# aynik/carta1

Hardware: AMD Instinct MI355X
Metric: atrac1_stereo_frames_per_s_encode (higher is better)
Workload: dtype f32+f64

## Files before the change

### carta1_amd/capi.py

```python
import ctypes as C
import os

HERE = os.path.dirname(os.path.abspath(__file__))
LIB_PATH = os.environ.get('C1_LIB') or os.path.join(HERE, 'lib', 'libcarta1_hip.so')

FRAME = 512
UNIT_BYTES = 212
SIGNAL_WHITE = 0
SIGNAL_PINK_BURSTS = 1
SIGNAL_MIXED = 2
SIGNAL_PARTIALS = 3


class Carta1Error(RuntimeError):
    def __init__(self, code, message):
        super().__init__('carta1_hip error %d: %s' % (code, message))
        self.code = code


class Tables(C.Structure):
    _fields_ = [('scale_factors', C.c_double * 64), ('window_short', C.c_double * 32),
                ('mdct_fwd64', C.c_double * 32), ('mdct_fwd256', C.c_double * 128),
                ('mdct_fwd512', C.c_double * 256), ('mdct_inv64', C.c_double * 32),
                ('mdct_inv256', C.c_double * 128), ('mdct_inv512', C.c_double * 256),
# ... 38 lines not shown
    'c1_dec_stream_create': (C.c_int, [C.c_void_p, C.c_int, C.POINTER(C.c_void_p)]),
    'c1_dec_stream_push': (C.c_int, [C.c_void_p, C.c_void_p, C.c_int64, C.POINTER(C.c_void_p)]),
    'c1_dec_stream_destroy': (C.c_int, [C.c_void_p]),
    'c1_generate_device': (C.c_int, [C.c_void_p, C.c_int, C.c_uint32, C.c_int64, C.c_void_p]),
    'c1_pcm_from_int_device': (C.c_int, [C.c_void_p, C.c_void_p, C.c_int, C.c_int, C.c_int64, C.POINTER(C.c_void_p)]),
    'c1_pcm_to_int16_device': (C.c_int, [C.c_void_p, C.POINTER(C.c_void_p), C.c_int, C.c_int64, C.c_void_p]),
    'c1_host_alloc': (C.c_int, [C.c_size_t, C.POINTER(C.c_void_p)]),
    'c1_host_free': (C.c_int, [C.c_void_p]),
    'c1_table_fast_paths': (C.c_int, [C.POINTER(C.c_int), C.POINTER(C.c_int)]),
    'c1_encode_wav_batch': (C.c_int, [C.c_void_p, C.c_void_p, C.c_int, C.c_int, C.c_int64, C.POINTER(EncodeOptions), C.c_void_p]),
    'c1_decode_wav16_batch': (C.c_int, [C.c_void_p, C.c_void_p, C.c_int, C.c_int64, C.c_void_p]),
    'c1_aea_header': (C.c_int, [C.c_char_p, C.c_uint32, C.c_int, C.c_void_p]),
    'c1_encode_stages_device': (C.c_int, [C.c_void_p, C.POINTER(C.c_void_p), C.c_int, C.c_int64, C.c_int,
                                          C.POINTER(EncodeOptions), C.c_void_p, C.c_void_p, C.c_void_p,
                                          C.c_void_p]),
    'c1_detect_stages_device': (C.c_int, [C.c_void_p, C.POINTER(C.c_void_p), C.c_int, C.c_int64, C.c_int,
                                          C.POINTER(EncodeOptions), C.c_void_p, C.c_void_p]),
    'c1_libm_device': (C.c_int, [C.c_void_p, C.c_int, C.c_void_p, C.c_void_p, C.c_int64]),
    'c1_detect_scores_device': (C.c_int, [C.c_void_p, C.POINTER(C.c_void_p), C.c_int, C.c_int64, C.c_int,
                                          C.POINTER(EncodeOptions), C.c_int, C.c_void_p, C.c_void_p, C.c_void_p]),
    'c1_detect_spec_mags_device': (C.c_int, [C.c_void_p, C.POINTER(C.c_void_p), C.c_int, C.c_int64, C.c_int, C.c_void_p, C.c_void_p]),
    'c1_log2f_error_device': (C.c_int, [C.c_void_p, C.c_uint32, C.c_uint64, C.POINTER(C.c_double)]),
    'c1_ctx_detection_stats': (C.c_int, [C.c_void_p, C.POINTER(C.c_uint64), C.POINTER(C.c_uint64)]),
    'c1_alloc_bounds_device': (C.c_int, [C.c_void_p, C.c_void_p, C.c_int64, C.c_void_p, C.c_void_p]),
    'c1_spec_stages_device': (C.c_int, [C.c_void_p, C.POINTER(C.c_void_p), C.c_int, C.c_int64, C.c_int,
                                        C.POINTER(EncodeOptions), C.c_void_p, C.c_void_p, C.c_void_p]),
    'c1_quantize': (C.c_int, [C.c_void_p, C.c_void_p, C.c_int, C.c_int, C.c_int, C.c_void_p]),
    'c1_dequantize': (C.c_int, [C.c_void_p, C.c_void_p, C.c_int, C.c_int, C.c_int, C.c_void_p]),
    'c1_fft': (C.c_int, [C.c_void_p, C.c_void_p, C.c_void_p, C.c_int, C.c_void_p]),
    'c1_qmf_analysis_batch': (C.c_int, [C.c_void_p, C.c_void_p, C.c_int64, C.c_int, C.c_void_p]),
    'c1_mdct_batch': (C.c_int, [C.c_void_p, C.c_void_p, C.c_int64, C.c_int, C.c_void_p, C.c_void_p, C.c_void_p]),
    'c1_unpack_units': (C.c_int, [C.c_void_p, C.c_void_p, C.c_int64, C.c_void_p, C.c_void_p, C.c_void_p, C.c_void_p, C.c_void_p]),
    'c1_dequantize_frames': (C.c_int, [C.c_void_p, C.c_int64, C.c_void_p, C.c_void_p, C.c_void_p, C.c_void_p, C.c_void_p, C.c_void_p]),
    'c1_imdct_batch': (C.c_int, [C.c_void_p, C.c_void_p, C.c_int64, C.c_int, C.c_void_p, C.c_void_p]),
    'c1_qmf_synthesis_batch': (C.c_int, [C.c_void_p, C.c_void_p, C.c_int64, C.c_int, C.c_void_p]),
    'c1_select_block_modes': (C.c_int, [C.c_void_p, C.c_void_p, C.c_int64, C.c_int, C.c_double, C.c_void_p]),
    'c1_quantize_frames': (C.c_int, [C.c_void_p, C.c_void_p, C.c_int64, C.c_void_p, C.c_void_p, C.c_void_p, C.c_void_p,
                                     C.c_void_p, C.c_void_p]),
    'c1_pack_spec_tap_device': (C.c_int, [C.c_void_p, C.c_void_p, C.c_void_p, C.c_void_p, C.c_void_p, C.c_int64, C.c_int,
                                          C.c_void_p, C.c_void_p]),
}

_lib = None


def load():
# ... 38 lines not shown
```

### carta1_amd/codec.py

```python
import ctypes as C
import math
import struct

import numpy as np

from . import capi

AEA_HEADER_SIZE = 2048
AEA_MAGIC = bytes([0x00, 0x08, 0x00, 0x00])
AEA_TITLE_OFFSET, AEA_TITLE_SIZE = 4, 256
AEA_FRAME_COUNT_OFFSET, AEA_CHANNEL_COUNT_OFFSET = 260, 264
BFU_AMOUNTS = (20, 28, 32, 36, 40, 44, 48, 52)
SPECS_PER_BFU = (8, 8, 8, 8, 4, 4, 4, 4, 8, 8, 8, 8, 6, 6, 6, 6, 6, 6, 6, 6, 6, 6, 6, 6, 7, 7, 7, 7, 9, 9, 9, 9,
                 10, 10, 10, 10, 12, 12, 12, 12, 12, 12, 12, 12, 20, 20, 20, 20, 20, 20, 20, 20)
WORD_LENGTH_BITS = (0, 2, 3, 4, 5, 6, 7, 8, 9, 10, 11, 12, 13, 14, 15, 16)


_BIASED = None


def packaged_biased_table(bias):
    global _BIASED
    if _BIASED is None:
        import json
# ... 81 lines not shown
        capi.check(capi.load().c1_ctx_kernel_ms(self._h, name.encode(), C.byref(ms), C.byref(n)))
        return ms.value, n.value

    def set_speculation(self, mode):
        capi.check(capi.load().c1_ctx_set_speculation(self._h, int(mode)))

    def set_decode_precision(self, binary32):
        capi.check(capi.load().c1_ctx_set_decode_precision(self._h, 1 if binary32 else 0))

    def speculation_stats(self, reset=False):
        u, r = C.c_uint64(0), C.c_uint64(0)
        capi.check(capi.load().c1_ctx_speculation_stats(self._h, C.byref(u), C.byref(r), 1 if reset else 0))
        return u.value, r.value

    def speculation_deferred(self):
        u = C.c_uint64(0)
        capi.check(capi.load().c1_ctx_speculation_deferred(self._h, C.byref(u)))
        return int(u.value)

    def quantization_stats(self):
        u, r = C.c_uint64(0), C.c_uint64(0)
        capi.check(capi.load().c1_ctx_quantization_stats(self._h, C.byref(u), C.byref(r)))
        return int(u.value), int(r.value)

    def detection_stats(self):
        u, r = C.c_uint64(0), C.c_uint64(0)
        capi.check(capi.load().c1_ctx_detection_stats(self._h, C.byref(u), C.byref(r)))
        return int(u.value), int(r.value)

    def encode(self, channels, options=None, halo_frames=0, out=None):
        opts = (options or EncoderOptions()).to_c()
        chans = [np.ascontiguousarray(c, dtype=np.float32) for c in channels]
        n = len(chans[0])
        if any(len(c) != n for c in chans) or n % 512:
            raise ValueError('channels must have equal length, a multiple of 512')
        frames = n // 512 - halo_frames
        if out is None:
            units = np.zeros((max(frames, 0) * len(chans), 212), dtype=np.uint8)
        else:
            units = out
            if units.dtype != np.uint8 or not units.flags['C_CONTIGUOUS'] or units.size != max(frames, 0) * len(chans) * 212:
                raise ValueError('out must be a contiguous uint8 array of frames * channels * 212 bytes')
            units = units.reshape(-1, 212)
        ptrs = capi.ptr_array([c.ctypes.data + halo_frames * 512 * 4 for c in chans])
        capi.check(capi.load().c1_encode_batch(self._h, ptrs, len(chans), frames, halo_frames, C.byref(opts),
                                               units.ctypes.data))
# ... 430 lines not shown
```

### carta1_amd/csrc/c1_api.hip

```cpp
#include <algorithm>
#include <cmath>
#include <cstdarg>
#include <cstdio>
#include <cstdlib>
#include <cstring>
#include <map>
#include <memory>
#include <atomic>
#include <mutex>
#include <string>
#include <thread>
#include <vector>

#include "c1_internal.h"
#include "c1_detect_bound.h"

#pragma clang fp contract(off)

namespace {

#include "c1_default_tables.inc"

thread_local std::string g_error;
int fail(int code, const char *fmt, ...) {
// ... 270 lines not shown
      for (int wl = 0; wl < 15; wl++) order.push_back(s * 16 + wl);
    std::sort(order.begin(), order.end(), [&](int x, int y) { return d->rank[x] < d->rank[y]; });
    for (int A = 1; A <= 12 && !d->rank_affine; A++)
      for (int B = 1; B <= 36 && !d->rank_affine; B++)
        for (int C = -2 * B; C <= 0 && !d->rank_affine; C++) {
          auto key = [&](int idx) { const int s = idx >> 4, wl = idx & 15; return wl == 0 ? A * s + C : A * s - B * wl - B; };
          bool ok = true;
          int lo = key(order[0]), hi = lo;
          for (size_t i = 1; i < order.size() && ok; i++) {
            const int k0 = key(order[i - 1]), k1 = key(order[i]);
            const bool req = d->rank[order[i]] == d->rank[order[i - 1]];
            if (req ? (k1 != k0) : !(k1 > k0)) ok = false;
            lo = std::min(lo, k1); hi = std::max(hi, k1);
          }
          if (ok && hi - lo + 1 < 1023) {
            d->rank_affine = 1; d->rank_a = A; d->rank_b = B; d->rank_c = C; d->rank_off = 1 - lo;
          }
        }
  }
  return C1_OK;
}

constexpr int kTotals = 8;
constexpr int64_t kSpecMinUnits = 64;
constexpr int kListHead = 8;
constexpr int64_t kMaxChunkFrames = (int64_t)1 << 27;

struct Timing {
  hipEvent_t start, stop;
  int kind;
};
enum { K_ANALYSIS = 0, K_ALLOCATE, K_PACK, K_DECODE, K_REDO, K_KINDS };
const char *const kKindNames[K_KINDS] = {"analysis", "allocate", "pack", "decode", "redo"};

}

struct c1_ctx {
  std::recursive_mutex mu;
  int device = 0;
  hipStream_t stream = nullptr;
  bool own_stream = false;
  C1DevTables *d_tables = nullptr;
  C1DevEncOpts *d_opts = nullptr;
  c1_encode_options last_opts;
  bool have_opts = false;
  int64_t ws_units = 0;
  float *d_coefs[2] = {nullptr, nullptr};
  uint8_t *d_side[2] = {nullptr, nullptr};
  uint8_t *d_alloc[2] = {nullptr, nullptr};
  uint8_t *d_cand[2] = {nullptr, nullptr};
  uint32_t *d_work[2] = {nullptr, nullptr};
  float *d_eps[2] = {nullptr, nullptr};
  uint32_t *d_redo[2] = {nullptr, nullptr};
  unsigned long long *d_spec_totals = nullptr;
  int spec_mode = 1;
  float spec_defer = 1.0f;
  bool decode_binary32 = false;
  bool spec_tables_ok = false;
  int64_t det_units = 0;
  float *d_bands[2] = {nullptr, nullptr};
  double *d_feat[2] = {nullptr, nullptr};
  uint8_t *d_modes[2] = {nullptr, nullptr};
  uint32_t *d_lists[2] = {nullptr, nullptr};
  bool overlap = false;
  hipStream_t s_tail = nullptr;
  hipEvent_t ev_main[2] = {nullptr, nullptr}, ev_tail[2] = {nullptr, nullptr};
  bool tail_used[2] = {false, false};
  bool tail_pending = false;
  int ws_next = 0;
  int64_t chunk_frames = 0;
  bool pipeline = true;
  hipStream_t s_ana = nullptr, s_rest = nullptr;
  hipEvent_t ev_in = nullptr, ev_ana[2] = {nullptr, nullptr}, ev_free[2] = {nullptr, nullptr}, ev_end[2] = {nullptr, nullptr};
  int timing_depth = 0;
  bool profiling = false;
  std::vector<Timing> timings;
  std::vector<hipEvent_t> event_pool;
  double ms[K_KINDS] = {0, 0, 0, 0, 0};
  int launches[K_KINDS] = {0, 0, 0, 0, 0};
// ... 113 lines not shown
}
void bind_defer(c1_ctx *ctx, int p, C1EncodeLaunch *L) {
  L->defer_list = ctx->d_redo[p] + kListHead + 3 * (size_t)ctx->ws_units;
}

int ensure_io(c1_ctx *ctx, size_t bytes) {
  if (bytes <= ctx->d_io_bytes) return C1_OK;
  if (ctx->d_io) hipFree(ctx->d_io);
  ctx->d_io = nullptr; ctx->d_io_bytes = 0;
  HIP_TRY(hipMalloc(&ctx->d_io, bytes));
  ctx->d_io_bytes = bytes;
  return C1_OK;
}

int upload_opts(c1_ctx *ctx, const c1_encode_options *opts) {
  if (!opts) return fail(C1_ERR_ARG, "options are NULL");
  if (ctx->have_opts && memcmp(&ctx->last_opts, opts, sizeof *opts) == 0) return C1_OK;
  C1DevEncOpts h;
  const int rc = build_encode_opts(*opts, &h);
  if (rc) return rc;
  int jr = join_tail(ctx);
  if (jr) return jr;
  HIP_TRY(hipStreamSynchronize(ctx->stream));
  HIP_TRY(hipMemcpy(ctx->d_opts, &h, sizeof h, hipMemcpyHostToDevice));
  ctx->last_opts = *opts;
  ctx->have_opts = true;
  return C1_OK;
}

hipEvent_t take_event(c1_ctx *ctx) {
  if (!ctx->event_pool.empty()) {
    hipEvent_t e = ctx->event_pool.back();
    ctx->event_pool.pop_back();
    return e;
  }
  hipEvent_t e;
  hipEventCreateWithFlags(&e, hipEventDisableSystemFence);
  return e;
}
struct ScopedTiming {
  c1_ctx *ctx;
  Timing t;
  bool on;
  hipStream_t stream;
  ScopedTiming(c1_ctx *c, int kind, hipStream_t s = nullptr) : ctx(c), on(c->profiling), stream(s ? s : c->stream) {
    if (!on) return;
// ... 77 lines not shown
    HIP_TRY(hipStreamWaitEvent(sA, ctx->ev_in, 0));
    HIP_TRY(hipStreamWaitEvent(sB, ctx->ev_in, 0));
  }
  int64_t index = 0;
  for (int64_t f0 = 0, n = 0; f0 < frames; f0 += n, ++index) {
    n = taps ? frames : std::min(chunk, frames - f0);
    int p = piped ? (int)(index & 1) : 0;
    if (overlap) { p = ctx->ws_next; ctx->ws_next ^= 1; }
    C1EncodeLaunch L;
    memset(&L, 0, sizeof L);
    for (int c = 0; c < channels; c++) L.pcm[c] = pcm[c] + f0 * 512;
    L.channels = channels;
    L.frames = n;
    L.halo_frames = (int)std::min<int64_t>(2, f0 + halo_frames);
    L.tables = ctx->d_tables;
    L.opts = ctx->d_opts;
    L.coefs = taps ? coefs_tap : ctx->d_coefs[p];
    L.side = taps ? side_tap : ctx->d_side[p];
    L.alloc = taps ? alloc_tap : ctx->d_alloc[p];
    L.cand = ctx->d_cand[p];
    L.work_count = ctx->d_work[p];
    L.work_list = ctx->d_work[p] + 4;
    L.sel_list = ctx->d_work[p] + 4 + (size_t)ctx->ws_units * 7;
    L.bands = bands ? bands + f0 * channels * 512 : nullptr;
    L.units = units ? units + f0 * channels * C1_UNIT_BYTES : nullptr;
    const bool all_long = all_long_modes;
    if (piped && index >= 2) HIP_TRY(hipStreamWaitEvent(sA, ctx->ev_free[p], 0));
    if (speculate) {
      L.eps = ctx->d_eps[p];
      bind_lists(ctx, p, &L);
      if (ctx->spec_mode == 1) { bind_defer(ctx, p, &L); L.spec_defer = ctx->spec_defer; }
      if (c1k_pick_run(n, channels, 0) <= 64 && !getenv("C1_NO_SF_PREPASS"))
        L.open_masks = reinterpret_cast<unsigned long long *>((reinterpret_cast<uintptr_t>(ctx->d_redo[p] + kListHead + 3 * (size_t)ctx->ws_units + (size_t)ctx->ws_units / 4 + 4) + 7) & ~(uintptr_t)7);
      if (overlap && ctx->tail_used[p]) HIP_TRY(hipStreamWaitEvent(sA, ctx->ev_tail[p], 0));
      HIP_TRY(hipMemsetAsync(ctx->d_redo[p], 0, kListHead * sizeof(uint32_t), sA));
      {
        ScopedTiming t(ctx, K_ANALYSIS, sA);
        c1k_launch_analysis_spec(L, all_short_modes, sA);
        if (L.defer_list) {
          C1EncodeLaunch D = L;
          uint32_t *dense = ctx->d_redo[p] + kListHead + 2 * (size_t)ctx->ws_units;
          c1k_launch_defer_compact(L, dense, ctx->d_redo[p] + 3, sA);
          D.unit_list = dense;
          D.unit_count = ctx->d_redo[p] + 3;
          D.list_runs = 1;
          D.defer_list = nullptr;
// ... 208 lines not shown
    const hipError_t se = hipStreamCreateWithFlags(&ctx->stream, hipStreamNonBlocking);
    if (se != hipSuccess) { delete ctx; return fail(C1_ERR_HIP, "hipStreamCreate: %s", hipGetErrorString(se)); }
    ctx->own_stream = true;
  }
  c1_tables t;
  {
    std::lock_guard<std::mutex> lock(g_tables_mutex);
    if (g_tables_custom) t = g_tables; else default_tables(&t);
  }
  C1DevTables *h = new C1DevTables();
  build_device_tables(t, h);
  hipError_t me = hipMalloc(&ctx->d_tables, sizeof(C1DevTables));
  if (me == hipSuccess) me = hipMalloc(&ctx->d_opts, sizeof(C1DevEncOpts));
  if (me == hipSuccess) me = hipMemcpy(ctx->d_tables, h, sizeof *h, hipMemcpyHostToDevice);
  if (me == hipSuccess) me = hipMalloc(&ctx->d_spec_totals, kTotals * sizeof(unsigned long long));
  if (me == hipSuccess) me = hipMemset(ctx->d_spec_totals, 0, kTotals * sizeof(unsigned long long));
  ctx->spec_tables_ok = h->spec_ok != 0;
  {
    const char *sp = getenv("C1_SPEC");
    ctx->spec_mode = sp ? atoi(sp) : 1;
    if (ctx->spec_mode < 0 || ctx->spec_mode > 2) ctx->spec_mode = 1;
    const char *sd = getenv("C1_SPEC_DEFER");
    if (sd && atof(sd) > 0) ctx->spec_defer = (float)atof(sd);
  }
  delete h;
  if (me != hipSuccess) { c1_ctx_destroy(ctx); return fail(C1_ERR_HIP, "table upload: %s", hipGetErrorString(me)); }
  {
    hipError_t pe = hipStreamCreateWithFlags(&ctx->s_ana, hipStreamNonBlocking);
    if (pe == hipSuccess) pe = hipStreamCreateWithFlags(&ctx->s_rest, hipStreamNonBlocking);
    if (pe == hipSuccess) pe = hipEventCreateWithFlags(&ctx->ev_in, hipEventDisableTiming);
    for (int p = 0; p < 2 && pe == hipSuccess; p++) {
      pe = hipEventCreateWithFlags(&ctx->ev_ana[p], hipEventDisableTiming);
      if (pe == hipSuccess) pe = hipEventCreateWithFlags(&ctx->ev_free[p], hipEventDisableTiming);
      if (pe == hipSuccess) pe = hipEventCreateWithFlags(&ctx->ev_end[p], hipEventDisableTiming);
    }
    if (pe != hipSuccess) { c1_ctx_destroy(ctx); return fail(C1_ERR_HIP, "pipeline streams: %s", hipGetErrorString(pe)); }
    if (pe == hipSuccess) pe = hipStreamCreateWithFlags(&ctx->s_tail, hipStreamNonBlocking);
    for (int p = 0; p < 2 && pe == hipSuccess; p++) {
      pe = hipEventCreateWithFlags(&ctx->ev_main[p], hipEventDisableTiming);
      if (pe == hipSuccess) pe = hipEventCreateWithFlags(&ctx->ev_tail[p], hipEventDisableTiming);
    }
    if (pe != hipSuccess) { c1_ctx_destroy(ctx); return fail(C1_ERR_HIP, "tail stream: %s", hipGetErrorString(pe)); }
    const char *ov = getenv("C1_OVERLAP");
    ctx->overlap = ov ? atoi(ov) != 0 : false;
    const char *pl = getenv("C1_PIPELINE");
    ctx->pipeline = pl ? atoi(pl) != 0 : false;
// ... 79 lines not shown
  CTX_GUARD(ctx);
  int rc = ctx_bind(ctx);
  if (rc) return rc;
  unsigned long long tot[2] = {0, 0};
  HIP_TRY(hipMemcpyAsync(tot, ctx->d_spec_totals, sizeof tot, hipMemcpyDeviceToHost, ctx->stream));
  HIP_TRY(hipStreamSynchronize(ctx->stream));
  if (units) *units = tot[0];
  if (redone) *redone = tot[1];
  if (reset) {
    HIP_TRY(hipMemsetAsync(ctx->d_spec_totals, 0, kTotals * sizeof(unsigned long long), ctx->stream));
    HIP_TRY(hipStreamSynchronize(ctx->stream));
  }
  return C1_OK;
}

int c1_ctx_speculation_deferred(c1_ctx *ctx, uint64_t *units) {
  CTX_GUARD(ctx);
  int rc = ctx_bind(ctx);
  if (rc) return rc;
  unsigned long long tot[kTotals];
  HIP_TRY(hipMemcpyAsync(tot, ctx->d_spec_totals, sizeof tot, hipMemcpyDeviceToHost, ctx->stream));
  HIP_TRY(hipStreamSynchronize(ctx->stream));
  if (units) *units = tot[6];
  return C1_OK;
}

int c1_ctx_quantization_stats(c1_ctx *ctx, uint64_t *units, uint64_t *repacked) {
  CTX_GUARD(ctx);
  int rc = ctx_bind(ctx);
  if (rc) return rc;
  unsigned long long tot[4] = {0, 0, 0, 0};
  HIP_TRY(hipMemcpyAsync(tot, ctx->d_spec_totals, sizeof tot, hipMemcpyDeviceToHost, ctx->stream));
  HIP_TRY(hipStreamSynchronize(ctx->stream));
  if (units) *units = tot[2];
  if (repacked) *repacked = tot[3];
  return C1_OK;
}

int c1_ctx_detection_stats(c1_ctx *ctx, uint64_t *units, uint64_t *rechecked) {
  CTX_GUARD(ctx);
  int rc = ctx_bind(ctx);
  if (rc) return rc;
  unsigned long long tot[6] = {0, 0, 0, 0, 0, 0};
  HIP_TRY(hipMemcpyAsync(tot, ctx->d_spec_totals, sizeof tot, hipMemcpyDeviceToHost, ctx->stream));
  HIP_TRY(hipStreamSynchronize(ctx->stream));
  if (units) *units = tot[4];
// ... 1241 lines not shown
```

### carta1_amd/csrc/c1_internal.h

```cpp
#pragma once

#include <hip/hip_runtime.h>
#include <stdint.h>
#include <stdlib.h>

#include "../../include/carta1_hip.h"

struct C1DevTables {
  double tap_e[24];
  double tap_o[24];
  double window[32];
  double mdct_fwd64[32];
  double mdct_fwd256[128];
  double mdct_fwd512[256];
  double mdct_inv64[32];
  double mdct_inv256[128];
  double mdct_inv512[256];
  double fft_tw[256][2];
  double scale_factors[64];
  double norm[64 * 16];
  double log1p10;
  uint32_t sf_m1, sf_m2;
  int32_t sf_fast;
  int32_t dq_fast;
// ... 8 lines not shown
  float r4b[4][3][2];
  float r4c[16][3][2];
  float r2d[64][2];
  float norm32[64 * 16];
  float inv32_64[16][2], inv32_256[64][2], inv32_512[128][2];
  float tw32[256][2];
  float spec_cz[4], spec_cw[4], spec_cl[4];
  float spec_cz_short[4], spec_cw_short[4], spec_cl_short[4];
  float spec_eabs;
  float det_ck[4];
  float det_eabs;
  int32_t spec_ok;
};

struct C1DevEncOpts {
  double biased[64];
  double threshold;
  int32_t modes[3];
  int32_t pad_;
  uint16_t rank[64 * 16];
  int32_t rank_affine, rank_a, rank_b, rank_c, rank_off;
  float la_slope, la_off;
  int32_t alloc_no_tonal;
};

constexpr int kRunFrames = 16;
constexpr int kRunFramesDecode = 64;
constexpr int kRunFramesLong = 64;
constexpr int kSideBytes = 64;
constexpr int kAllocBytes = 32;
constexpr int kCandidateBytes = 8 * 8 + 8 * 32 + 8 * 8;
constexpr int kCandLbOffset = 8 * 8 + 8 * 32;
constexpr int kEpsFloats = 4;
constexpr uint32_t kEpsFlagSfOpen = 1u;
constexpr uint32_t kEpsFlagExact = 2u;
constexpr int kSpecCheckFrames = 16;

struct C1EncodeLaunch {
  const float *pcm[C1_MAX_CHANNELS];
  int channels;
  int64_t frames;
  int halo_frames;
  const C1DevTables *tables;
  const C1DevEncOpts *opts;
  float *coefs;
  uint8_t *side;
  uint8_t *alloc;
  uint8_t *cand;
  uint32_t *work_list;
  uint32_t *work_count;
  uint32_t *sel_list;
  float *bands;
  float *mags;
  float *mag_bounds;
  uint8_t *units;
  float *eps;
  uint32_t *redo_list;
  uint32_t *redo_count;
  uint32_t *realloc_list;
  uint32_t *realloc_count;
  uint32_t *reana_list;
  uint32_t *reana_count;
  uint32_t *defer_list;
  unsigned long long *open_masks;
  int list_zero_eps;
  float spec_defer;
  const uint32_t *unit_list;
  const uint32_t *unit_count;
  int list_runs;
  int run_frames;
  int spread_bits;
};

// ... 71 lines not shown
```

### carta1_amd/csrc/c1_k_allocate.hip

```cpp
#include "c1_device.h"

namespace {

constexpr int kHeapSlotsPerLane = 52 + 1;
constexpr uint32_t kLow = 0x1FFFFFu;
constexpr uint32_t kSentinel = 52u;
constexpr int kCandBytes = kCandidateBytes;
constexpr double kAlive = -1.0;

__device__ __forceinline__ uint32_t heap_entry(uint32_t rank, int size, int s, int wl, int b) {
  return (rank << 21) | ((uint32_t)size << 16) | ((uint32_t)s << 10) | ((uint32_t)wl << 6) | (uint32_t)b;
}

__device__ __forceinline__ void heap_sift_down(uint32_t *hp, int sentinel, int i, uint32_t v, uint32_t el,
                                               uint32_t er, bool active) {
  const uint32_t vmax = v | kLow;
  for (;;) {
    const uint32_t m = max(el | kLow, vmax);
    const bool take_r = er > m;
    const bool take_l = !take_r && el > vmax;
    const bool moved = active && (take_r || take_l);
    if (active) hp[i * 64] = moved ? (take_r ? er : el) : v;
    active = moved;
    if (__builtin_amdgcn_ballot_w64(active) == 0) break;
    i = moved ? 2 * i + 1 + (take_r ? 1 : 0) : i;
    const int l = 2 * i + 1;
    const uint32_t *src = hp + min(l, sentinel - 1) * 64;
    el = l < sentinel ? src[0] : 0u;
    er = src[64];
  }
}

__device__ __forceinline__ void run_candidate(uint32_t *hp, int n, const uint32_t (&sf)[13], const C1DevEncOpts *O,
                                              bool live, uint64_t &res0, uint64_t &res1, uint64_t &res2,
                                              uint64_t &res3, double &total) {
  const __attribute__((address_space(4))) uint16_t *rank_t = (const __attribute__((address_space(4))) uint16_t *)O->rank;
  const __attribute__((address_space(4))) double *biased = (const __attribute__((address_space(4))) double *)O->biased;
  const bool affine = O->rank_affine != 0;
  const int ka = O->rank_a, kb = O->rank_b, kc = O->rank_c, koff = O->rank_off;
  const int nkb = -kb, kc_off = kc + koff;
  auto rank_of = [&](int s, int wl) -> uint32_t {
    if (affine) return (uint32_t)(wl == 0 ? __mul24(ka, s) + kc_off : __mul24(ka, s) + koff + __mul24(nkb, wl + 1));
    return rank_t[s * 16 + (wl & 15)];
  };
  int remaining = 212 * 8 - 40 - 10 * n;
  int hs = 0;
#pragma unroll
  for (int b = 0; b < 52; b++) {
    if (b < n) {
      const int s = (sf[b >> 2] >> ((b & 3) * 8)) & 63;
      hp[hs * 64] = heap_entry(rank_of(s, 0), kSpecs[b], s, 0, b);
      hs += (s != 0 && live) ? 1 : 0;
    }
  }
  for (int k = hs; k < kHeapSlotsPerLane; k++) hp[k * 64] = kSentinel;
  for (int i = (hs >> 1) - 1; i >= 0; i--) {
    const int l = 2 * i + 1;
    heap_sift_down(hp, 52, i, hp[i * 64], hp[l * 64], hp[(l + 1) * 64], true);
  }
  uint32_t r0 = hp[0], r1 = hp[64], r2 = hp[128];
  bool run = remaining >= 4 && hs > 0;
  while (__builtin_amdgcn_ballot_w64(run) != 0) {
    const uint32_t top = r0;
    const int wl = (top >> 6) & 15, size = (top >> 16) & 31, s = (top >> 10) & 63;
    const int cost = size << (wl == 0 ? 1 : 0);
    const bool fits = cost <= remaining;
    const int nxt = wl + (fits ? 1 : 0);
    const bool leaves = run && (!fits || nxt >= 15);
    const uint32_t upd = (top & ~((0x3FFu << 21) | (15u << 6))) | ((uint32_t)nxt << 6);
    uint32_t v = upd | (rank_of(s, nxt) << 21);
    if (__builtin_amdgcn_ballot_w64(leaves) != 0) {
      const int li = hs - 1;
      const uint32_t deep = hp[(li > 3 ? li : 3) * 64];
      const uint32_t last = li == 0 ? r0 : (li == 1 ? r1 : (li == 2 ? r2 : deep));
      if (leaves) {
        v = last;
        hs = li;
        if (li > 2) hp[li * 64] = upd;
        r0 = li == 0 ? upd : r0; r1 = li == 1 ? upd : r1; r2 = li == 2 ? upd : r2;
      }
    }
    if (run) remaining -= fits ? cost : 0;
    const bool sift = run && hs > 0;
    const uint32_t vmax = v | kLow;
    const bool tr0 = r2 > max(r1 | kLow, vmax);
// ... 19 lines not shown
        if (mv1) hp[i2 * 64] = mv2 ? (tr2 ? c1 : c0) : v;
        if (__builtin_amdgcn_ballot_w64(mv2) != 0) {
          const int i3 = 2 * i2 + 1 + (tr2 ? 1 : 0);
          const uint32_t *s3 = hp + (2 * i3 + 1) * 64;
          const uint32_t d0 = s3[0], d1 = s3[64];
          const int q = 4 * i3 + 3;
          const uint32_t h0 = hp[min(q, 52) * 64], h1 = hp[min(q + 1, 52) * 64], h2 = hp[min(q + 2, 52) * 64], h3 = hp[min(q + 3, 52) * 64];
          const bool tr3 = d1 > max(d0 | kLow, vmax);
          const bool tl3 = !tr3 && d0 > vmax;
          const bool mv3 = mv2 && (tr3 || tl3);
          if (mv2) hp[i3 * 64] = mv3 ? (tr3 ? d1 : d0) : v;
          const int i4 = 2 * i3 + 1 + (tr3 ? 1 : 0);
          const uint32_t e0 = tr3 ? h2 : h0, e1 = tr3 ? h3 : h1;
          const bool tr4 = e1 > max(e0 | kLow, vmax);
          const bool tl4 = !tr4 && e0 > vmax;
          const bool mv4 = mv3 && (tr4 || tl4);
          if (mv3) hp[i4 * 64] = mv4 ? (tr4 ? e1 : e0) : v;
          if (mv4) hp[(2 * i4 + 1 + (tr4 ? 1 : 0)) * 64] = v;
        }
      }
    }
    run = run && remaining >= 4 && hs > 0;
  }
  hp[0] = r0; hp[64] = r1; hp[128] = r2;
  {
    uint8_t *hb = reinterpret_cast<uint8_t *>(hp);
#pragma unroll
    for (int k = 0; k < 52; k++) hb[k * 256 + 3] = 0;
#pragma unroll
    for (int k0 = 0; k0 < 52; k0 += 8) {
      uint32_t e[8];
#pragma unroll
      for (int j = 0; j < 8; j++) if (k0 + j < 52) e[j] = hp[(k0 + j) * 64];
#pragma unroll
      for (int j = 0; j < 8; j++) if (k0 + j < 52) hb[(e[j] & 63u) * 256 + 3] = (uint8_t)((e[j] >> 6) & 15u);
    }
    uint32_t d[8];
#pragma unroll
    for (int i = 0; i < 8; i++) {
      d[i] = 0;
#pragma unroll
      for (int j = 0; j < 8; j++) if (8 * i + j < 52) d[i] |= (hp[(8 * i + j) * 64] >> 24) << (4 * j);
    }
    res0 = (uint64_t)d[0] | ((uint64_t)d[1] << 32); res1 = (uint64_t)d[2] | ((uint64_t)d[3] << 32);
    res2 = (uint64_t)d[4] | ((uint64_t)d[5] << 32); res3 = (uint64_t)d[6] | ((uint64_t)d[7] << 32);
  }
  total = 0.0;
#pragma unroll
  for (int b = 0; b < 52; b++) {
    const int s = (sf[b >> 2] >> ((b & 3) * 8)) & 63;
    const uint64_t word = b < 16 ? res0 : (b < 32 ? res1 : (b < 48 ? res2 : res3));
    const int wl = (int)((word >> ((b & 15) * 4)) & 15);
    const int size = kSpecs[b];
    const double bs = biased[s];
    if (b >= n || wl == 0) {
      total += s != 0 ? (double)f32(bs * 2.0 * (double)size) : 0.0;
    } else if (s != 0) {
      const double ip2 = __hiloint2double((1023 - wl_bits(wl)) << 20, 0);
      total += bs * ip2 * (double)size;
    }
  }
}

__device__ __forceinline__ void load_sfi(const uint8_t *side, int64_t unit, uint32_t (&sf)[13]) {
  const uint4 *src = reinterpret_cast<const uint4 *>(side + unit * kSideBytes);
  const uint4 a = src[0], b = src[1], c = src[2];
  const uint32_t d = reinterpret_cast<const uint32_t *>(src)[12];
  sf[0] = a.x; sf[1] = a.y; sf[2] = a.z; sf[3] = a.w; sf[4] = b.x; sf[5] = b.y; sf[6] = b.z; sf[7] = b.w;
  sf[8] = c.x; sf[9] = c.y; sf[10] = c.z; sf[11] = c.w; sf[12] = d;
}

__device__ __forceinline__ void store_candidate(uint8_t *cand, int64_t unit, int c, double total, uint64_t r0,
                                                uint64_t r1, uint64_t r2, uint64_t r3) {
  uint8_t *base = cand + unit * kCandBytes;
  reinterpret_cast<double *>(base)[c] = total;
  uint64_t *dst = reinterpret_cast<uint64_t *>(base + 64 + c * 32);
  dst[0] = r0; dst[1] = r1; dst[2] = r2; dst[3] = r3;
}

__device__ __forceinline__ bool getenv_no_tonal(const C1DevEncOpts *O) { return O->alloc_no_tonal != 0; }

__global__ __launch_bounds__(C1_WAVE, 3) void k_alloc_first(C1EncodeLaunch L) {
  __shared__ uint32_t heap[kHeapSlotsPerLane * 64];
  const C1DevEncOpts *O = L.opts;
  const __attribute__((address_space(4))) double *biased = (const __attribute__((address_space(4))) double *)O->biased;
  const int lane = threadIdx.x;
  const bool listed = L.unit_list != nullptr;
  const int64_t units_total = listed ? (int64_t)*L.unit_count : L.frames * L.channels;
  for (int64_t pos0 = (int64_t)blockIdx.x * 64; pos0 < units_total; pos0 += (int64_t)gridDim.x * 64) {
  const int64_t pos = pos0 + lane;
  const bool live = pos < units_total;
  const int64_t unit = listed ? (int64_t)L.unit_list[live ? pos : 0] : pos;
  uint32_t sf[13];
  load_sfi(L.side, live ? unit : 0, sf);
  bool tonal = false;
  {
    float n_coef = 0.0f, s_la = 0.0f;
#pragma unroll
    for (int b = 0; b < 52; b++) {
      const int s = (sf[b >> 2] >> ((b & 3) * 8)) & 63;
      const float w = s != 0 ? (float)kSpecs[b] : 0.0f;
      n_coef += w;
      s_la = __builtin_fmaf(w, (float)s, s_la);
    }
    const float la_sum = __builtin_fmaf(O->la_slope, s_la, O->la_off * n_coef);
    const float t_est = 1.442695f * n_coef * __builtin_amdgcn_exp2f((la_sum - 1136.0f) / n_coef);
    float t6f = 0.0f;
#pragma unroll
    for (int b = 48; b < 52; b++) {
      const int s = (sf[b >> 2] >> ((b & 3) * 8)) & 63;
      const float bs = (float)biased[s];
      t6f += s != 0 ? bs * (2.0f * (float)kSpecs[b]) : 0.0f;
    }
    const bool mine = n_coef > 0.0f && t6f < 0.35f * t_est && !getenv_no_tonal(O);
    tonal = 2 * __popcll(__builtin_amdgcn_ballot_w64(live && mine)) > __popcll(__builtin_amdgcn_ballot_w64(live));
  }
  uint64_t r0, r1, r2, r3;
  double total;
  run_candidate(heap + lane, 52, sf, O, live && !tonal, r0, r1, r2, r3, total);
  uint32_t survivors = 0;
  {
    double t0 = 0, t1 = 0, t2 = 0, t3 = 0, t4 = 0, t5 = 0, t6 = 0;
#pragma unroll
    for (int b = 20; b < 52; b++) {
      const int s = (sf[b >> 2] >> ((b & 3) * 8)) & 63;
      const double bs = biased[s];
      const double z = s != 0 ? (double)f32(bs * 2.0 * (double)kSpecs[b]) : 0.0;
      t0 += z;
      if (b >= 28) t1 += z;
      if (b >= 32) t2 += z;
      if (b >= 36) t3 += z;
      if (b >= 40) t4 += z;
      if (b >= 44) t5 += z;
      if (b >= 48) t6 += z;
    }
    const bool finite = total < __builtin_huge_val();
    survivors = (!(finite && t0 > total) ? 1u : 0u) | (!(finite && t1 > total) ? 2u : 0u) |
                (!(finite && t2 > total) ? 4u : 0u) | (!(finite && t3 > total) ? 8u : 0u) |
                (!(finite && t4 > total) ? 16u : 0u) | (!(finite && t5 > total) ? 32u : 0u) |
                (!(finite && t6 > total) ? 64u : 0u);
  }
  if (tonal) survivors = 0xffu;
  const bool finite52 = total < __builtin_huge_val();
  if (live && survivors == 0) {
    uint64_t *dst = reinterpret_cast<uint64_t *>(L.alloc + unit * kAllocBytes);
    if (finite52) { dst[0] = r0; dst[1] = r1; dst[2] = r2; dst[3] = r3 | (7ull << 60); }
    else { dst[0] = 0; dst[1] = 0; dst[2] = 0; dst[3] = 1ull << 59; }
  } else if (live) {
    uint8_t *base = L.cand + unit * kCandBytes;
    double *tot = reinterpret_cast<double *>(base);
#pragma unroll
    for (int c = 0; c < 7; c++) tot[c] = ((survivors >> c) & 1u) ? kAlive : __builtin_huge_val();
    if (tonal) tot[7] = kAlive;
    else store_candidate(L.cand, unit, 7, finite52 ? total : __builtin_huge_val(), r0, r1, r2, r3);
  }
  const uint64_t sel_mask = __builtin_amdgcn_ballot_w64(live && survivors != 0);
  uint32_t sel_base = 0;
  if (lane == 0 && sel_mask != 0) sel_base = atomicAdd(L.work_count + 1, (uint32_t)__popcll(sel_mask));
  sel_base = (uint32_t)__builtin_amdgcn_readfirstlane((int)sel_base);
  if (live && survivors != 0) L.sel_list[sel_base + (uint32_t)__popcll(sel_mask & ((1ull << lane) - 1ull))] = (uint32_t)unit;
  }
}

typedef _Float16 h2 __attribute__((ext_vector_type(2)));
constexpr int kSpecsHost[52] = {8, 8, 8, 8, 4, 4, 4, 4, 8, 8, 8, 8, 6, 6, 6, 6, 6, 6, 6, 6, 6, 6, 6, 6, 7, 7, 7, 7, 9, 9, 9, 9, 10, 10, 10, 10,
                                12, 12, 12, 12, 12, 12, 12, 12, 20, 20, 20, 20, 20, 20, 20, 20};
__global__ __launch_bounds__(256) void k_alloc_bound(C1EncodeLaunch L) {
  __shared__ double biased_s[64];
  const C1DevEncOpts *O = L.opts;
  if (threadIdx.x < 64) biased_s[threadIdx.x] = threadIdx.x == 0 ? 0.0 : ((const __attribute__((address_space(4))) double *)O->biased)[threadIdx.x];
  __syncthreads();
  const float la_slope = O->la_slope, la_off = O->la_off;
  const int lane = threadIdx.x & 63;
  const uint32_t count = L.work_count[1];
  for (uint32_t pos0 = blockIdx.x * 256u; pos0 < count; pos0 += gridDim.x * 256u) {
    const uint32_t pos = pos0 + threadIdx.x;
    const bool live = pos < count;
    const int64_t unit = live ? (int64_t)L.sel_list[pos] : (int64_t)L.sel_list[0];
    uint32_t sf[13];
    load_sfi(L.side, unit, sf);
    uint8_t *base = L.cand + unit * kCandBytes;
    double *tot = reinterpret_cast<double *>(base);
    double *lb = reinterpret_cast<double *>(base + kCandLbOffset);
// ... 173 lines not shown
  const uint32_t a7 = reinterpret_cast<const uint32_t *>(L.alloc + unit * kAllocBytes)[7];
  out[unit * 16 + 15] = ((a7 >> 27) & 1u) ? -1.0 : (double)((a7 >> 28) & 7u);
}

}

void c1k_launch_alloc_tap(const C1EncodeLaunch &L, double *out, hipStream_t stream) {
  const int64_t units = L.frames * L.channels;
  c1k_launch_allocate(L, stream);
  const dim3 grid((unsigned)((units + 255) / 256)), block(256);
  hipLaunchKernelGGL(k_alloc_tap_init, grid, block, 0, stream, L, units);
  hipLaunchKernelGGL(k_alloc_bound, dim3((unsigned)std::min<int64_t>((units + 255) / 256, 2048)), block, 0, stream, L);
  hipLaunchKernelGGL((k_alloc_rest<false>), dim3((unsigned)std::min<int64_t>((units * 8 + 63) / 64, 256 * 10)), dim3(C1_WAVE), 0, stream, L,
                     (const uint32_t *)(L.work_list + units), (const uint32_t *)(L.work_count + 2), (uint32_t *)nullptr);
  hipLaunchKernelGGL(k_alloc_tap_gather, grid, block, 0, stream, L, units, out);
}

namespace {
}

void c1k_launch_allocate(const C1EncodeLaunch &L, hipStream_t stream) {
  const int64_t units = L.frames * L.channels;
  const bool listed = L.unit_list != nullptr;
  (void)hipMemsetAsync(L.work_count, 0, 3 * sizeof(uint32_t), stream);
  const int64_t first_blocks = listed ? std::min<int64_t>((units + 63) / 64, 256 * 12) : (units + 63) / 64;
  hipLaunchKernelGGL(k_alloc_first, dim3((unsigned)first_blocks), dim3(C1_WAVE), 0, stream, L);
  const int64_t unit_blocks = std::min<int64_t>((units + 255) / 256, 2048);
  uint32_t *list2 = L.work_list + units;
  hipLaunchKernelGGL(k_alloc_bound, dim3((unsigned)unit_blocks), dim3(256), 0, stream, L);
  const int64_t rest1_blocks = std::min<int64_t>((units + 63) / 64, 256 * 10);
  hipLaunchKernelGGL((k_alloc_rest<true>), dim3((unsigned)rest1_blocks), dim3(C1_WAVE), 0, stream, L, (const uint32_t *)L.work_list, (const uint32_t *)L.work_count, list2);
  const int64_t rest2_blocks = std::min<int64_t>((units * 6 + 63) / 64, 256 * 10);
  hipLaunchKernelGGL((k_alloc_rest<false>), dim3((unsigned)rest2_blocks), dim3(C1_WAVE), 0, stream, L, (const uint32_t *)list2, (const uint32_t *)(L.work_count + 2), (uint32_t *)nullptr);
  const int64_t select_blocks = std::min<int64_t>((units + 255) / 256, 1024);
  hipLaunchKernelGGL(k_alloc_select, dim3((unsigned)select_blocks), dim3(256), 0, stream, L);
}
```

### include/carta1_hip.h

```cpp
#ifndef CARTA1_HIP_H
#define CARTA1_HIP_H

#include <stddef.h>
#include <stdint.h>

#ifdef __cplusplus
extern "C" {
#endif

#define C1_FRAME_SAMPLES 512
#define C1_UNIT_BYTES 212
#define C1_MAX_CHANNELS 2
#define C1_ABI_VERSION 3

enum {
  C1_OK = 0,
  C1_ERR_ARG = 1,
  C1_ERR_NO_DEVICE = 2,
  C1_ERR_HIP = 3,
  C1_ERR_STATE = 4
};

typedef struct c1_tables {
  double scale_factors[64];
// ... 16 lines not shown
} c1_encode_options;

typedef struct c1_ctx c1_ctx;

int c1_abi_version(void);
const char *c1_last_error(void);
int c1_device_count(int *count);
int c1_get_default_tables(c1_tables *out);
int c1_set_tables(const c1_tables *tables);
int c1_default_encode_options(c1_encode_options *out);
int c1_table_fast_paths(int *scale_factor_bits, int *dequant_reciprocal);

int c1_ctx_create(int device, void *hip_stream , c1_ctx **out);
int c1_ctx_destroy(c1_ctx *ctx);
int c1_ctx_synchronize(c1_ctx *ctx);
int c1_ctx_set_profiling(c1_ctx *ctx, int enabled);
int c1_ctx_kernel_ms(c1_ctx *ctx, const char *name, double *ms, int *launches);

int c1_ctx_set_speculation(c1_ctx *ctx, int mode);
int c1_ctx_speculation_stats(c1_ctx *ctx, uint64_t *units, uint64_t *redone, int reset);
int c1_ctx_speculation_deferred(c1_ctx *ctx, uint64_t *units);
int c1_ctx_quantization_stats(c1_ctx *ctx, uint64_t *units, uint64_t *repacked);
int c1_ctx_detection_stats(c1_ctx *ctx, uint64_t *units, uint64_t *rechecked);

int c1_ctx_set_decode_precision(c1_ctx *ctx, int binary32);


int c1_encode_device(c1_ctx *ctx, const float *const *pcm, int channels, int64_t frames,
                     int halo_frames, const c1_encode_options *opts, uint8_t *units);
int c1_encode_batch(c1_ctx *ctx, const float *const *pcm, int channels, int64_t frames,
                    int halo_frames, const c1_encode_options *opts, uint8_t *units);

int c1_encode_batch_multi(const int *devices, int n_devices, const float *const *pcm, int channels, int64_t frames,
                          int halo_frames, const c1_encode_options *opts, uint8_t *units);
int c1_decode_batch_multi(const int *devices, int n_devices, const uint8_t *units, int channels, int64_t frames,
                          int halo_units, float *const *pcm);

int c1_host_alloc(size_t bytes, void **out);
int c1_host_free(void *p);

int c1_decode_device(c1_ctx *ctx, const uint8_t *units, int channels, int64_t frames,
                     int halo_units, float *const *pcm);
int c1_decode_batch(c1_ctx *ctx, const uint8_t *units, int channels, int64_t frames,
                    int halo_units, float *const *pcm);

typedef struct c1_enc_stream c1_enc_stream;
// ... 70 lines not shown
```

Measured before the change: 182.2 million.

## Park straggler lanes' heap allocation state and resume them in a compacted kernel

The first allocation kernel now stops its wave-wide greedy heap loop once at most a configurable number of lanes (default 8) are still running. The parked lanes write their heap state into the candidate record, and a new k_alloc_resume kernel finishes them in densely packed waves. The goal is to cut the divergence where a whole 64-lane wave keeps iterating for a few long-running units. The cost is an extra kernel launch, global-memory spills and reloads of the heap state, and an extra counter and stats API.

```diff
diff --git a/carta1_amd/capi.py b/carta1_amd/capi.py
--- a/carta1_amd/capi.py
+++ b/carta1_amd/capi.py
@@ -84,6 +84,7 @@
     'c1_detect_spec_mags_device': (C.c_int, [C.c_void_p, C.POINTER(C.c_void_p), C.c_int, C.c_int64, C.c_int, C.c_void_p, C.c_void_p]),
     'c1_log2f_error_device': (C.c_int, [C.c_void_p, C.c_uint32, C.c_uint64, C.POINTER(C.c_double)]),
     'c1_ctx_detection_stats': (C.c_int, [C.c_void_p, C.POINTER(C.c_uint64), C.POINTER(C.c_uint64)]),
+    'c1_ctx_allocation_stats': (C.c_int, [C.c_void_p, C.POINTER(C.c_uint64)]),
     'c1_alloc_bounds_device': (C.c_int, [C.c_void_p, C.c_void_p, C.c_int64, C.c_void_p, C.c_void_p]),
     'c1_spec_stages_device': (C.c_int, [C.c_void_p, C.POINTER(C.c_void_p), C.c_int, C.c_int64, C.c_int,
                                         C.POINTER(EncodeOptions), C.c_void_p, C.c_void_p, C.c_void_p]),
diff --git a/carta1_amd/codec.py b/carta1_amd/codec.py
--- a/carta1_amd/codec.py
+++ b/carta1_amd/codec.py
@@ -127,6 +127,11 @@
         u, r = C.c_uint64(0), C.c_uint64(0)
         capi.check(capi.load().c1_ctx_quantization_stats(self._h, C.byref(u), C.byref(r)))
         return int(u.value), int(r.value)
+
+    def allocation_stats(self):
+        u = C.c_uint64(0)
+        capi.check(capi.load().c1_ctx_allocation_stats(self._h, C.byref(u)))
+        return int(u.value)
 
     def detection_stats(self):
         u, r = C.c_uint64(0), C.c_uint64(0)
diff --git a/carta1_amd/csrc/c1_api.hip b/carta1_amd/csrc/c1_api.hip
--- a/carta1_amd/csrc/c1_api.hip
+++ b/carta1_amd/csrc/c1_api.hip
@@ -316,6 +316,7 @@
 }
 
 constexpr int kTotals = 8;
+constexpr int kAllocParkDefault = 8;
 constexpr int64_t kSpecMinUnits = 64;
 constexpr int kListHead = 8;
 constexpr int64_t kMaxChunkFrames = (int64_t)1 << 27;
@@ -349,6 +350,7 @@
   unsigned long long *d_spec_totals = nullptr;
   int spec_mode = 1;
   float spec_defer = 1.0f;
+  int alloc_park = kAllocParkDefault;
   bool decode_binary32 = false;
   bool spec_tables_ok = false;
   int64_t det_units = 0;
@@ -508,6 +510,7 @@
   int jr = join_tail(ctx);
   if (jr) return jr;
   HIP_TRY(hipStreamSynchronize(ctx->stream));
+  h.alloc_park = ctx->alloc_park;
   HIP_TRY(hipMemcpy(ctx->d_opts, &h, sizeof h, hipMemcpyHostToDevice));
   ctx->last_opts = *opts;
   ctx->have_opts = true;
@@ -631,6 +634,7 @@
     L.work_count = ctx->d_work[p];
     L.work_list = ctx->d_work[p] + 4;
     L.sel_list = ctx->d_work[p] + 4 + (size_t)ctx->ws_units * 7;
+    L.park_total = ctx->d_spec_totals + 7;
     L.bands = bands ? bands + f0 * channels * 512 : nullptr;
     L.units = units ? units + f0 * channels * C1_UNIT_BYTES : nullptr;
     const bool all_long = all_long_modes;
@@ -885,6 +889,8 @@
     if (ctx->spec_mode < 0 || ctx->spec_mode > 2) ctx->spec_mode = 1;
     const char *sd = getenv("C1_SPEC_DEFER");
     if (sd && atof(sd) > 0) ctx->spec_defer = (float)atof(sd);
+    const char *pk = getenv("C1_ALLOC_PARK");
+    if (pk) ctx->alloc_park = std::min(63, std::max(0, atoi(pk)));
   }
   delete h;
   if (me != hipSuccess) { c1_ctx_destroy(ctx); return fail(C1_ERR_HIP, "table upload: %s", hipGetErrorString(me)); }
@@ -1010,6 +1016,17 @@
   HIP_TRY(hipMemcpyAsync(tot, ctx->d_spec_totals, sizeof tot, hipMemcpyDeviceToHost, ctx->stream));
   HIP_TRY(hipStreamSynchronize(ctx->stream));
   if (units) *units = tot[6];
+  return C1_OK;
+}
+
+int c1_ctx_allocation_stats(c1_ctx *ctx, uint64_t *parked) {
+  CTX_GUARD(ctx);
+  int rc = ctx_bind(ctx);
+  if (rc) return rc;
+  unsigned long long tot[kTotals];
+  HIP_TRY(hipMemcpyAsync(tot, ctx->d_spec_totals, sizeof tot, hipMemcpyDeviceToHost, ctx->stream));
+  HIP_TRY(hipStreamSynchronize(ctx->stream));
+  if (parked) *parked = tot[7];
   return C1_OK;
 }
 
diff --git a/carta1_amd/csrc/c1_internal.h b/carta1_amd/csrc/c1_internal.h
--- a/carta1_amd/csrc/c1_internal.h
+++ b/carta1_amd/csrc/c1_internal.h
@@ -54,6 +54,7 @@
   int32_t rank_affine, rank_a, rank_b, rank_c, rank_off;
   float la_slope, la_off;
   int32_t alloc_no_tonal;
+  int32_t alloc_park;
 };
 
 constexpr int kRunFrames = 16;
@@ -81,6 +82,7 @@
   uint8_t *cand;
   uint32_t *work_list;
   uint32_t *work_count;
+  unsigned long long *park_total;
   uint32_t *sel_list;
   float *bands;
   float *mags;
diff --git a/carta1_amd/csrc/c1_k_allocate.hip b/carta1_amd/csrc/c1_k_allocate.hip
--- a/carta1_amd/csrc/c1_k_allocate.hip
+++ b/carta1_amd/csrc/c1_k_allocate.hip
@@ -7,6 +7,8 @@
 constexpr uint32_t kSentinel = 52u;
 constexpr int kCandBytes = kCandidateBytes;
 constexpr double kAlive = -1.0;
+constexpr int kParkDwords = 56;
+static_assert(kParkDwords * 4 <= kCandBytes && kParkDwords >= kHeapSlotsPerLane + 2, "parked heap state must fit a candidate record");
 
 __device__ __forceinline__ uint32_t heap_entry(uint32_t rank, int size, int s, int wl, int b) {
   return (rank << 21) | ((uint32_t)size << 16) | ((uint32_t)s << 10) | ((uint32_t)wl << 6) | (uint32_t)b;
@@ -31,20 +33,23 @@
   }
 }
 
-__device__ __forceinline__ void run_candidate(uint32_t *hp, int n, const uint32_t (&sf)[13], const C1DevEncOpts *O,
-                                              bool live, uint64_t &res0, uint64_t &res1, uint64_t &res2,
-                                              uint64_t &res3, double &total) {
-  const __attribute__((address_space(4))) uint16_t *rank_t = (const __attribute__((address_space(4))) uint16_t *)O->rank;
-  const __attribute__((address_space(4))) double *biased = (const __attribute__((address_space(4))) double *)O->biased;
-  const bool affine = O->rank_affine != 0;
-  const int ka = O->rank_a, kb = O->rank_b, kc = O->rank_c, koff = O->rank_off;
-  const int nkb = -kb, kc_off = kc + koff;
-  auto rank_of = [&](int s, int wl) -> uint32_t {
+struct HeapRank {
+  const __attribute__((address_space(4))) uint16_t *t;
+  bool affine;
+  int ka, nkb, koff, kc_off;
+  __device__ __forceinline__ explicit HeapRank(const C1DevEncOpts *O)
+      : t((const __attribute__((address_space(4))) uint16_t *)O->rank),
+        affine(O->rank_affine != 0), ka(O->rank_a), nkb(-O->rank_b), koff(O->rank_off), kc_off(O->rank_c + O->rank_off) {}
+  __device__ __forceinline__ uint32_t operator()(int s, int wl) const {
     if (affine) return (uint32_t)(wl == 0 ? __mul24(ka, s) + kc_off : __mul24(ka, s) + koff + __mul24(nkb, wl + 1));
-    return rank_t[s * 16 + (wl & 15)];
-  };
-  int remaining = 212 * 8 - 40 - 10 * n;
-  int hs = 0;
+    return t[s * 16 + (wl & 15)];
+  }
+};
+
+__device__ __forceinline__ void heap_build(uint32_t *hp, int n, const uint32_t (&sf)[13], const HeapRank &rank_of, bool live,
+                                           int &remaining, int &hs) {
+  remaining = 212 * 8 - 40 - 10 * n;
+  hs = 0;
 #pragma unroll
   for (int b = 0; b < 52; b++) {
     if (b < n) {
@@ -58,9 +63,12 @@
     const int l = 2 * i + 1;
     heap_sift_down(hp, 52, i, hp[i * 64], hp[l * 64], hp[(l + 1) * 64], true);
   }
-  uint32_t r0 = hp[0], r1 = hp[64], r2 = hp[128];
+}
+
+__device__ __forceinline__ bool heap_spend(uint32_t *hp, const HeapRank &rank_of, uint32_t &r0, uint32_t &r1, uint32_t &r2,
+                                           int &remaining, int &hs, int park) {
   bool run = remaining >= 4 && hs > 0;
-  while (__builtin_amdgcn_ballot_w64(run) != 0) {
+  while (__popcll(__builtin_amdgcn_ballot_w64(run)) > park) {
     const uint32_t top = r0;
     const int wl = (top >> 6) & 15, size = (top >> 16) & 31, s = (top >> 10) & 63;
     const int cost = size << (wl == 0 ? 1 : 0);
@@ -126,6 +134,13 @@
     }
     run = run && remaining >= 4 && hs > 0;
   }
+  return run;
+}
+
+__device__ __forceinline__ void heap_result(uint32_t *hp, int n, const uint32_t (&sf)[13], const C1DevEncOpts *O, uint32_t r0,
+                                            uint32_t r1, uint32_t r2, uint64_t &res0, uint64_t &res1, uint64_t &res2,
+                                            uint64_t &res3, double &total) {
+  const __attribute__((address_space(4))) double *biased = (const __attribute__((address_space(4))) double *)O->biased;
   hp[0] = r0; hp[64] = r1; hp[128] = r2;
   {
     uint8_t *hb = reinterpret_cast<uint8_t *>(hp);
@@ -166,6 +181,17 @@
   }
 }
 
+__device__ __forceinline__ void run_candidate(uint32_t *hp, int n, const uint32_t (&sf)[13], const C1DevEncOpts *O,
+                                              bool live, uint64_t &res0, uint64_t &res1, uint64_t &res2,
+                                              uint64_t &res3, double &total) {
+  const HeapRank rank_of(O);
+  int remaining, hs;
+  heap_build(hp, n, sf, rank_of, live, remaining, hs);
+  uint32_t r0 = hp[0], r1 = hp[64], r2 = hp[128];
+  heap_spend(hp, rank_of, r0, r1, r2, remaining, hs, 0);
+  heap_result(hp, n, sf, O, r0, r1, r2, res0, res1, res2, res3, total);
+}
+
 __device__ __forceinline__ void load_sfi(const uint8_t *side, int64_t unit, uint32_t (&sf)[13]) {
   const uint4 *src = reinterpret_cast<const uint4 *>(side + unit * kSideBytes);
   const uint4 a = src[0], b = src[1], c = src[2];
@@ -183,6 +209,53 @@
 }
 
 __device__ __forceinline__ bool getenv_no_tonal(const C1DevEncOpts *O) { return O->alloc_no_tonal != 0; }
+
+__device__ __forceinline__ void finish_first(const C1EncodeLaunch &L, int lane, int64_t unit, bool live, bool tonal,
+                                             const uint32_t (&sf)[13], uint64_t r0, uint64_t r1, uint64_t r2, uint64_t r3,
+                                             double total) {
+  const __attribute__((address_space(4))) double *biased = (const __attribute__((address_space(4))) double *)L.opts->biased;
+  uint32_t survivors = 0;
+  {
+    double t0 = 0, t1 = 0, t2 = 0, t3 = 0, t4 = 0, t5 = 0, t6 = 0;
+#pragma unroll
+    for (int b = 20; b < 52; b++) {
+      const int s = (sf[b >> 2] >> ((b & 3) * 8)) & 63;
+      const double bs = biased[s];
+      const double z = s != 0 ? (double)f32(bs * 2.0 * (double)kSpecs[b]) : 0.0;
+      t0 += z;
+      if (b >= 28) t1 += z;
+      if (b >= 32) t2 += z;
+      if (b >= 36) t3 += z;
+      if (b >= 40) t4 += z;
+      if (b >= 44) t5 += z;
+      if (b >= 48) t6 += z;
+    }
+    const bool finite = total < __builtin_huge_val();
+    survivors = (!(finite && t0 > total) ? 1u : 0u) | (!(finite && t1 > total) ? 2u : 0u) |
+                (!(finite && t2 > total) ? 4u : 0u) | (!(finite && t3 > total) ? 8u : 0u) |
+                (!(finite && t4 > total) ? 16u : 0u) | (!(finite && t5 > total) ? 32u : 0u) |
+                (!(finite && t6 > total) ? 64u : 0u);
+  }
+  if (tonal) survivors = 0xffu;
+  const bool finite52 = total < __builtin_huge_val();
+  if (live && survivors == 0) {
+    uint64_t *dst = reinterpret_cast<uint64_t *>(L.alloc + unit * kAllocBytes);
+    if (finite52) { dst[0] = r0; dst[1] = r1; dst[2] = r2; dst[3] = r3 | (7ull << 60); }
+    else { dst[0] = 0; dst[1] = 0; dst[2] = 0; dst[3] = 1ull << 59; }
+  } else if (live) {
+    uint8_t *base = L.cand + unit * kCandBytes;
+    double *tot = reinterpret_cast<double *>(base);
+#pragma unroll
+    for (int c = 0; c < 7; c++) tot[c] = ((survivors >> c) & 1u) ? kAlive : __builtin_huge_val();
+    if (tonal) tot[7] = kAlive;
+    else store_candidate(L.cand, unit, 7, finite52 ? total : __builtin_huge_val(), r0, r1, r2, r3);
+  }
+  const uint64_t sel_mask = __builtin_amdgcn_ballot_w64(live && survivors != 0);
+  uint32_t sel_base = 0;
+  if (lane == 0 && sel_mask != 0) sel_base = atomicAdd(L.work_count + 1, (uint32_t)__popcll(sel_mask));
+  sel_base = (uint32_t)__builtin_amdgcn_readfirstlane((int)sel_base);
+  if (live && survivors != 0) L.sel_list[sel_base + (uint32_t)__popcll(sel_mask & ((1ull << lane) - 1ull))] = (uint32_t)unit;
+}
 
 __global__ __launch_bounds__(C1_WAVE, 3) void k_alloc_first(C1EncodeLaunch L) {
   __shared__ uint32_t heap[kHeapSlotsPerLane * 64];
@@ -219,50 +292,78 @@
     const bool mine = n_coef > 0.0f && t6f < 0.35f * t_est && !getenv_no_tonal(O);
     tonal = 2 * __popcll(__builtin_amdgcn_ballot_w64(live && mine)) > __popcll(__builtin_amdgcn_ballot_w64(live));
   }
+  const HeapRank rank_of(O);
+  uint32_t *hp = heap + lane;
+  int remaining, hs;
+  heap_build(hp, 52, sf, rank_of, live && !tonal, remaining, hs);
+  uint32_t h0 = hp[0], h1 = hp[64], h2 = hp[128];
+  const bool parked = heap_spend(hp, rank_of, h0, h1, h2, remaining, hs, listed ? 0 : O->alloc_park);
+  const uint64_t park_mask = __builtin_amdgcn_ballot_w64(parked);
+  if (park_mask != 0) {
+    uint32_t at = 0;
+    if (lane == 0) at = atomicAdd(L.work_count + 3, (uint32_t)__popcll(park_mask));
+    at = (uint32_t)__builtin_amdgcn_readfirstlane((int)at);
+    if (parked) {
+      uint4 *dst = reinterpret_cast<uint4 *>(L.cand + unit * kCandBytes);
+#pragma unroll
+      for (int k = 0; k < kParkDwords / 4; k++) {
+        uint32_t w[4];
+#pragma unroll
+        for (int j = 0; j < 4; j++) {
+          const int i = 4 * k + j;
+          w[j] = i == 0 ? h0 : i == 1 ? h1 : i == 2 ? h2 : i < kHeapSlotsPerLane ? hp[i * 64] : i == kHeapSlotsPerLane ? (uint32_t)remaining
+                 : i == kHeapSlotsPerLane + 1 ? (uint32_t)hs : 0u;
+        }
+        dst[k] = make_uint4(w[0], w[1], w[2], w[3]);
+      }
+      L.work_list[at + (uint32_t)__popcll(park_mask & ((1ull << lane) - 1ull))] = (uint32_t)unit;
+    }
+  }
   uint64_t r0, r1, r2, r3;
   double total;
-  run_candidate(heap + lane, 52, sf, O, live && !tonal, r0, r1, r2, r3, total);
-  uint32_t survivors = 0;
-  {
-    double t0 = 0, t1 = 0, t2 = 0, t3 = 0, t4 = 0, t5 = 0, t6 = 0;
-#pragma unroll
-    for (int b = 20; b < 52; b++) {
-      const int s = (sf[b >> 2] >> ((b & 3) * 8)) & 63;
-      const double bs = biased[s];
-      const double z = s != 0 ? (double)f32(bs * 2.0 * (double)kSpecs[b]) : 0.0;
-      t0 += z;
-      if (b >= 28) t1 += z;
-      if (b >= 32) t2 += z;
-      if (b >= 36) t3 += z;
-      if (b >= 40) t4 += z;
-      if (b >= 44) t5 += z;
-      if (b >= 48) t6 += z;
-    }
-    const bool finite = total < __builtin_huge_val();
-    survivors = (!(finite && t0 > total) ? 1u : 0u) | (!(finite && t1 > total) ? 2u : 0u) |
-                (!(finite && t2 > total) ? 4u : 0u) | (!(finite && t3 > total) ? 8u : 0u) |
-                (!(finite && t4 > total) ? 16u : 0u) | (!(finite && t5 > total) ? 32u : 0u) |
-                (!(finite && t6 > total) ? 64u : 0u);
-  }
-  if (tonal) survivors = 0xffu;
-  const bool finite52 = total < __builtin_huge_val();
-  if (live && survivors == 0) {
-    uint64_t *dst = reinterpret_cast<uint64_t *>(L.alloc + unit * kAllocBytes);
-    if (finite52) { dst[0] = r0; dst[1] = r1; dst[2] = r2; dst[3] = r3 | (7ull << 60); }
-    else { dst[0] = 0; dst[1] = 0; dst[2] = 0; dst[3] = 1ull << 59; }
-  } else if (live) {
-    uint8_t *base = L.cand + unit * kCandBytes;
-    double *tot = reinterpret_cast<double *>(base);
-#pragma unroll
-    for (int c = 0; c < 7; c++) tot[c] = ((survivors >> c) & 1u) ? kAlive : __builtin_huge_val();
-    if (tonal) tot[7] = kAlive;
-    else store_candidate(L.cand, unit, 7, finite52 ? total : __builtin_huge_val(), r0, r1, r2, r3);
-  }
-  const uint64_t sel_mask = __builtin_amdgcn_ballot_w64(live && survivors != 0);
-  uint32_t sel_base = 0;
-  if (lane == 0 && sel_mask != 0) sel_base = atomicAdd(L.work_count + 1, (uint32_t)__popcll(sel_mask));
-  sel_base = (uint32_t)__builtin_amdgcn_readfirstlane((int)sel_base);
-  if (live && survivors != 0) L.sel_list[sel_base + (uint32_t)__popcll(sel_mask & ((1ull << lane) - 1ull))] = (uint32_t)unit;
+  heap_result(hp, 52, sf, O, h0, h1, h2, r0, r1, r2, r3, total);
+  finish_first(L, lane, unit, live && !parked, tonal, sf, r0, r1, r2, r3, total);
+  }
+}
+
+__global__ __launch_bounds__(C1_WAVE, 3) void k_alloc_resume(C1EncodeLaunch L) {
+  __shared__ uint32_t heap[kHeapSlotsPerLane * 64];
+  const C1DevEncOpts *O = L.opts;
+  const int lane = threadIdx.x;
+  const uint32_t count = L.work_count[3];
+  if (blockIdx.x == 0 && lane == 0 && count != 0 && L.park_total) atomicAdd(L.park_total, (unsigned long long)count);
+  const HeapRank rank_of(O);
+  uint32_t *hp = heap + lane;
+  for (uint32_t pos0 = blockIdx.x * 64u; pos0 < count; pos0 += gridDim.x * 64u) {
+    const uint32_t pos = pos0 + lane;
+    const bool live = pos < count;
+    const int64_t unit = (int64_t)L.work_list[live ? pos : 0u];
+    uint32_t sf[13];
+    load_sfi(L.side, unit, sf);
+    const uint4 *src = reinterpret_cast<const uint4 *>(L.cand + unit * kCandBytes);
+    uint32_t h0 = kSentinel, h1 = kSentinel, h2 = kSentinel;
+    int remaining = 0, hs = 0;
+#pragma unroll
+    for (int k = 0; k < kParkDwords / 4; k++) {
+      const uint4 q = src[k];
+      const uint32_t w[4] = {q.x, q.y, q.z, q.w};
+#pragma unroll
+      for (int j = 0; j < 4; j++) {
+        const int i = 4 * k + j;
+        const uint32_t v = live ? w[j] : (i < kHeapSlotsPerLane ? kSentinel : 0u);
+        if (i < kHeapSlotsPerLane) hp[i * 64] = v;
+        if (i == 0) h0 = v;
+        if (i == 1) h1 = v;
+        if (i == 2) h2 = v;
+        if (i == kHeapSlotsPerLane) remaining = (int)v;
+        if (i == kHeapSlotsPerLane + 1) hs = (int)v;
+      }
+    }
+    heap_spend(hp, rank_of, h0, h1, h2, remaining, hs, 0);
+    uint64_t r0, r1, r2, r3;
+    double total;
+    heap_result(hp, 52, sf, O, h0, h1, h2, r0, r1, r2, r3, total);
+    finish_first(L, lane, unit, live, false, sf, r0, r1, r2, r3, total);
   }
 }
 
@@ -482,9 +583,10 @@
 void c1k_launch_allocate(const C1EncodeLaunch &L, hipStream_t stream) {
   const int64_t units = L.frames * L.channels;
   const bool listed = L.unit_list != nullptr;
-  (void)hipMemsetAsync(L.work_count, 0, 3 * sizeof(uint32_t), stream);
+  (void)hipMemsetAsync(L.work_count, 0, 4 * sizeof(uint32_t), stream);
   const int64_t first_blocks = listed ? std::min<int64_t>((units + 63) / 64, 256 * 12) : (units + 63) / 64;
   hipLaunchKernelGGL(k_alloc_first, dim3((unsigned)first_blocks), dim3(C1_WAVE), 0, stream, L);
+  if (!listed) hipLaunchKernelGGL(k_alloc_resume, dim3((unsigned)std::min<int64_t>((units + 63) / 64, 256 * 12)), dim3(C1_WAVE), 0, stream, L);
   const int64_t unit_blocks = std::min<int64_t>((units + 255) / 256, 2048);
   uint32_t *list2 = L.work_list + units;
   hipLaunchKernelGGL(k_alloc_bound, dim3((unsigned)unit_blocks), dim3(256), 0, stream, L);
diff --git a/include/carta1_hip.h b/include/carta1_hip.h
--- a/include/carta1_hip.h
+++ b/include/carta1_hip.h
@@ -62,6 +62,7 @@
 int c1_ctx_speculation_deferred(c1_ctx *ctx, uint64_t *units);
 int c1_ctx_quantization_stats(c1_ctx *ctx, uint64_t *units, uint64_t *repacked);
 int c1_ctx_detection_stats(c1_ctx *ctx, uint64_t *units, uint64_t *rechecked);
+int c1_ctx_allocation_stats(c1_ctx *ctx, uint64_t *parked);
 
 int c1_ctx_set_decode_precision(c1_ctx *ctx, int binary32);
 
```

New measurement: 183.7 million (median of 6 runs). Within noise of the previous version (+0.8%).
